# sarphiv/nerf-experiments

Hardware: AMD Instinct MI355X
Metric: ray-samples/sec (coarse+fine), training step (higher is better)
Workload: dtype fp32

## Files before the change

include/nerf_amd.h:

```cpp
#ifndef NERF_AMD_H
#define NERF_AMD_H

#include <stdint.h>
#include <stddef.h>

#ifdef __cplusplus
extern "C" {
#endif

#define NERF_OK 0
#define NERF_ERR_INVALID_ARG (-1)
#define NERF_ERR_UNSUPPORTED (-2)
#define NERF_ERR_LAUNCH (-3)
#define NERF_ERR_WORKSPACE (-4)

int nerf_abi_version(void);
const char* nerf_status_string(int status);
int64_t nerf_struct_size(int32_t which);
#define NERF_BUILD_DIAG_FUSED 1
#define NERF_BUILD_DIAG_WGRAD 2
int32_t nerf_build_flags(void);

int nerf_composite_fwd(const float* density, int64_t density_stride,
                       const float* color, int64_t color_stride,
// ... 145 lines not shown
    float* out2;
    int64_t ldo2;
    int32_t n1;
    int32_t hbm_off;
    int32_t seg_gen[2];
} nerf_fused_layer;

struct nerf_hashgrid_params;
typedef struct nerf_fused_encoding {
    nerf_pe_params params;
    const float* ray_o;
    const float* ray_d;
    const float* t_start;
    const float* t_end;
    const float* pixel_width;
    float* out;
    int64_t ld;
    int64_t n_rays;
    int32_t samples_per_ray;
    int32_t per_ray;
    int32_t out_dim;
    int32_t reserved;
    const struct nerf_hashgrid_params* hash;
    const float* hash_table;
} nerf_fused_encoding;

int nerf_mlp_fused_fwd(const nerf_fused_layer* layers, int32_t n_layers, const void* image, int64_t M,
                       const nerf_fused_encoding* encodings, void* stream);

typedef struct nerf_fused_composite {
    const float* dist;
    float* rgb;
    float* weights;
    float* coef;
    const float* grad_rgb;
    float* grad_head;
    int64_t ld_head;
    float* grad_sigma;
    int64_t ld_sigma;
    int32_t samples_per_ray;
    int32_t head_layer;
    int32_t sigma_layer;
    float scale_a, scale_b;
    float density_shift;
    int32_t reserved;
} nerf_fused_composite;

int nerf_mlp_fused_render(const nerf_fused_layer* layers, int32_t n_layers, const void* image, int64_t M,
                          const nerf_fused_encoding* encodings, const nerf_fused_composite* composite,
                          void* stream);

#define NERF_FUSED_BF16 1
#define NERF_FUSED_SPLIT_OUT(l) (1 << (8 + (l)))
int nerf_mlp_fused_run(const nerf_fused_layer* layers, int32_t n_layers, const void* image, int64_t M,
                       const nerf_fused_encoding* encodings, const nerf_fused_composite* composite, int32_t flags,
                       void* stream);

#define NERF_FUSED_MAX_SRCS 64
int nerf_fused_pack(const float* const* srcs, int32_t n_srcs, const int32_t* map_src, const int32_t* map_dst,
                    int64_t n, void* image, void* stream);

size_t nerf_gauss_act_workspace(int64_t M, int32_t N);

#define NERF_GAUSS_FWD 0
#define NERF_GAUSS_BWD 1
size_t nerf_linear_gauss_workspace(int64_t M, int32_t N);
int nerf_linear_gauss_x3(const nerf_seg* segs, int32_t n_segs, int64_t M, const void* W_x, int32_t ldw,
                         int32_t N, const float* bias, float* out, int64_t ldo, int32_t mode,
                         const float* inv_std, float* y, int64_t ld_y, const float* z, int64_t ld_z,
                         float* grad_inv_std, int32_t accumulate, void* workspace, size_t workspace_bytes,
                         void* stream);
int nerf_gauss_act_fwd(const float* z, int64_t ld_z, const float* inv_std, int64_t M, int32_t N,
                       float* y, int64_t ld_y, void* stream);
int nerf_gauss_act_bwd(const float* grad_y, int64_t ld_g, const float* z, int64_t ld_z,
                       const float* inv_std, int64_t M, int32_t N, float* grad_z, int64_t ld_dz,
                       float* grad_inv_std, int32_t accumulate, void* workspace, size_t workspace_bytes,
                       void* stream);

#define NERF_ACT_GABOR 1
#define NERF_ACT_SARF 2
size_t nerf_param_act_workspace(int32_t kind, int64_t M, int32_t N);
int nerf_param_act_fwd(int32_t kind, const float* z, int64_t ld_z, const float* p0, const float* p1, int64_t M,
                       int32_t N, float* y, int64_t ld_y, void* stream);
int nerf_param_act_bwd(int32_t kind, const float* grad_y, int64_t ld_g, const float* z, int64_t ld_z,
                       const float* p0, const float* p1, int64_t M, int32_t N, float* grad_z, int64_t ld_dz,
                       float* grad_p0, float* grad_p1, int32_t accumulate, void* workspace,
                       size_t workspace_bytes, void* stream);

size_t nerf_linear_act_workspace(int32_t kind, int64_t M, int32_t N);
int nerf_linear_act_x3(int32_t kind, const nerf_seg* segs, int32_t n_segs, int64_t M, const void* W_x, int32_t ldw,
                       int32_t N, const float* bias, float* out, int64_t ldo, int32_t mode, const float* p0,
                       const float* p1, float* y, int64_t ld_y, const float* z, int64_t ld_z, float* grad_p0,
                       float* grad_p1, int32_t accumulate, void* workspace, size_t workspace_bytes, void* stream);

#define NERF_ADAM_MAX_TENSORS 48
typedef struct nerf_adam_batch {
    int32_t n_tensors;
    float beta1, beta2, eps;
    float one_minus_beta1, one_minus_beta2;
    float* param[NERF_ADAM_MAX_TENSORS];
    const float* grad[NERF_ADAM_MAX_TENSORS];
    float* exp_avg[NERF_ADAM_MAX_TENSORS];
    float* exp_avg_sq[NERF_ADAM_MAX_TENSORS];
    int64_t numel[NERF_ADAM_MAX_TENSORS];
    float step_size[NERF_ADAM_MAX_TENSORS];
    float bc2_sqrt[NERF_ADAM_MAX_TENSORS];
// ... 76 lines not shown
```

nerf-experiments_amd/csrc/mlp_fused.hip:

```cpp
#include <stddef.h>
#include <stdlib.h>
#include <string.h>

#include <type_traits>

#include "common.h"
#include "encode_common.h"
#include "composite_common.h"
#include "hashgrid_common.h"

using namespace nerf;

typedef float f4 __attribute__((ext_vector_type(4)));
typedef float f8 __attribute__((ext_vector_type(8)));
typedef __bf16 bf16x8 __attribute__((ext_vector_type(8)));
typedef __bf16 bf16x4 __attribute__((ext_vector_type(4)));

namespace {

typedef __attribute__((address_space(3))) void lds_void_t;
typedef __attribute__((address_space(1))) void glb_void_t;

constexpr int SLOT_BYTES = 16 * 1024;
constexpr int NSLOT = 2;
constexpr int SB = 1;
constexpr int XIMG_BYTES = SB * 16 * 1024;
constexpr int WG = 512 / SB;
constexpr int NWAVE = WG / 64;
constexpr int SPW = 16 * SB;
constexpr int TILE = NWAVE * SPW;
constexpr int KBMAX = 8;
constexpr unsigned OOB = 0x80000000u;
constexpr int RSRC_W3 = 0x00020000;
constexpr int ST_AUX = 2;
constexpr bool is_fwd(int mode) { return (mode & 1) == 0; }
constexpr bool is_x1(int mode) { return (mode & 2) != 0; }
constexpr bool is_qs(int mode) { return (mode & 4) != 0; }
template <int MODE>
constexpr int after_dma_vm() { return is_fwd(MODE) ? 1 + 2 * SB : 2 * SB; }

struct FusedArgs {
    nerf_fused_layer L[NERF_FUSED_MAX_LAYERS];
    nerf_fused_encoding enc[2];
    const char* img;
    int img_bytes;
    int gen_mask;
    int gen_lds;
    int gen_reg;
    int n_layers;
    int M;
    int ntiles;
    int span;
    int comp_on;
    int split_mask;
    nerf_fused_composite comp;
    nerf_hashgrid_params hg;
    const float* hg_table;
    int hg_off[16];
};
static_assert(sizeof(FusedArgs) <= 4096, "kernel arguments");

typedef __attribute__((address_space(4))) const char kchar_t;
typedef float* fptr_t;
typedef const float* cfptr_t;
typedef uint8_t* u8ptr_t;
typedef const uint8_t* cu8ptr_t;
#define LF(T, f, l)                                                                                          \
    (*(const __attribute__((address_space(4))) T*)(c.kargs + offsetof(FusedArgs, L) +                        \
                                                   (size_t)(l) * sizeof(nerf_fused_layer) +                  \
                                                   offsetof(nerf_fused_layer, f)))
#define LFI(T, f, i, l)                                                                                      \
    (*(const __attribute__((address_space(4))) T*)(c.kargs + offsetof(FusedArgs, L) +                        \
                                                   (size_t)(l) * sizeof(nerf_fused_layer) +                  \
                                                   offsetof(nerf_fused_layer, f) + (size_t)(i) * sizeof(T)))

#define EF(T, f, e)                                                                                          \
    (*(const __attribute__((address_space(4))) T*)(c.kargs + offsetof(FusedArgs, enc) +                      \
                                                   (size_t)(e) * sizeof(nerf_fused_encoding) +               \
                                                   offsetof(nerf_fused_encoding, f)))

#define HG(T, f) (*(const __attribute__((address_space(4))) T*)(c.kargs + offsetof(FusedArgs, hg) +               \
                                                               offsetof(nerf_hashgrid_params, f)))

#define CF(T, f)                                                                                             \
    (*(const __attribute__((address_space(4))) T*)(c.kargs + offsetof(FusedArgs, comp) +                    \
                                                   offsetof(nerf_fused_composite, f)))

__device__ __forceinline__ f4 mfma16(bf16x8 a, bf16x8 b, f4 c) {
    return __builtin_amdgcn_mfma_f32_16x16x32_bf16(a, b, c, 0, 0, 0);
}
__device__ __forceinline__ void split8(f8 v, bf16x8& hi, bf16x8& lo) {
    hi = __builtin_convertvector(v, bf16x8);
    lo = __builtin_convertvector(v - __builtin_convertvector(hi, f8), bf16x8);
}

__device__ __forceinline__ void barrier() {
    asm volatile("s_waitcnt lgkmcnt(0)" ::: "memory");
    __builtin_amdgcn_s_barrier();
    __builtin_amdgcn_sched_barrier(0);
}

__device__ __forceinline__ int n16_of(int N) { return (N + 15) >> 4; }

__device__ __forceinline__ unsigned lds_addr(const void* p) {
    return (unsigned)(uintptr_t)(const __attribute__((address_space(3))) char*)p;
}
template <int OFF>
// ... 472 lines not shown
                f4 va, vb;
                unsigned oa, ob;
                pair_stores(c, st, sb, ch, st.colok, st.pa[sb], st.pb[sb], v, va, vb, oa, ob);
                __builtin_amdgcn_raw_buffer_store_b128(va, st.ro, oa, 0, ST_AUX);
                __builtin_amdgcn_raw_buffer_store_b128(vb, st.ro, ob, 0, ST_AUX);
            } else {
                f4 va, vb;
                unsigned oa, ob;
                pair_stores(c, st, sb, ch - st.n1, st.colok2, st.pa2[sb], st.pb2[sb], v, va, vb, oa, ob);
                __builtin_amdgcn_raw_buffer_store_b128(va, st.ro2, oa, 0, ST_AUX);
                __builtin_amdgcn_raw_buffer_store_b128(vb, st.ro2, ob, 0, ST_AUX);
            }
        }
    } else if (p == 2) {
        if constexpr (is_fwd(MODE)) {
            if (ch >= 0 && ch < 2 * KBMAX) {
#pragma unroll
                for (int sb = 0; sb < SB; ++sb) {
                    unsigned t = st.mw[sb][1];
#pragma unroll
                    for (int r = 3; r >= 0; --r) t = shift_in_dead(t, a[sb][r]);
                    st.mw[sb][1] = t;
                }
                if (ch == 7) {
#pragma unroll
                    for (int sb = 0; sb < SB; ++sb) {
                        st.mw[sb][0] = st.mw[sb][1];
                        st.mw[sb][1] = 0;
                    }
                }
            }
        }
    } else {
        if (ch >= 0 && ch < 2 * KBMAX && ch < st.n1 && !(is_qs(MODE) && st.qsplit)) {
#pragma unroll
            for (int sb = 0; sb < SB; ++sb) {
                typedef unsigned u2 __attribute__((ext_vector_type(2)));
                char* d = c.ximg + ((q * SB + sb) * 2) * 1024 + c.lane * 16 + 8 * bb;
                if constexpr (is_x1(MODE)) {
                    *reinterpret_cast<u2*>(d) = u2{hi2(a[sb][0], a[sb][1]), hi2(a[sb][2], a[sb][3])};
                } else {
                    unsigned h0, l0, h1, l1;
                    split2(a[sb][0], a[sb][1], h0, l0);
                    split2(a[sb][2], a[sb][3], h1, l1);
                    const u2 h = {h0, h1}, lo = {l0, l1};
                    *reinterpret_cast<u2*>(d) = h;
                    *reinterpret_cast<u2*>(d + 1024) = lo;
                }
            }
        }
    }
}

constexpr int EPI_NP = 3;
__host__ __device__ constexpr int epi_part_of(int i) {
    return i == 0 ? 0 : i + 1;
}
template <int KBR, int EPI0>
__host__ __device__ constexpr int epi_placed() {
    return KBR - EPI0 < EPI_NP ? (KBR - EPI0 > 0 ? KBR - EPI0 : 0) : EPI_NP;
}

template <int MODE>
constexpr int epi0_of() { return is_fwd(MODE) ? 3 : 4; }

constexpr int FA = 2;

template <int MODE, int KBR, int I>
__device__ __forceinline__ void first_reads(bf16x8 (&fr)[FA][2], unsigned sa) {
    if constexpr (I < FA && I < KBR) {
        lds_frag<I * 2048>(fr[I][0], sa);
        if constexpr (!is_x1(MODE)) lds_frag<I * 2048 + 1024>(fr[I][1], sa);
        first_reads<MODE, KBR, I + 1>(fr, sa);
    }
}

template <int MODE, int KBR, int KBH, int KB_I, int EPAR = -1>
__device__ __forceinline__ void reg_steps(Ctx& c, LayerState& st, unsigned sa, bf16x8 (&fr)[FA][2], f4 (&a)[SB],
                                          f4 (&pv)[SB], f4& pb, int ch) {
    constexpr int EPI0 = KBR >= 8 ? epi0_of<MODE>() : (KBR >= 4 ? 1 : 0);
    if constexpr (KB_I < KBR) {
        bf16x8(&f)[2] = fr[KB_I % FA];
        constexpr int later = (KB_I + FA - 1 < KBR - 1 ? KB_I + FA - 1 : KBR - 1) - KB_I;
        if constexpr (is_x1(MODE)) {
            lds_wait1<later>(f[0]);
#pragma unroll
            for (int sb = 0; sb < SB; ++sb) a[sb] = mfma16(f[0], c.xh[KB_I][sb], a[sb]);
        } else {
            lds_wait<2 * later>(f[0], f[1]);
#pragma unroll
            for (int sb = 0; sb < SB; ++sb) a[sb] = mfma16(f[1], c.xh[KB_I][sb], a[sb]);
#pragma unroll
            for (int sb = 0; sb < SB; ++sb) a[sb] = mfma16(f[0], c.xl[KB_I][sb], a[sb]);
#pragma unroll
            for (int sb = 0; sb < SB; ++sb) a[sb] = mfma16(f[0], c.xh[KB_I][sb], a[sb]);
        }
        if constexpr (KB_I + FA < KBR) {
            lds_frag<(KB_I + FA) * 2048>(f[0], sa);
            if constexpr (!is_x1(MODE)) lds_frag<(KB_I + FA) * 2048 + 1024>(f[1], sa);
        }
        if constexpr (KB_I == EPI0 && is_fwd(MODE))
            bias_wait<(KBR > 0 ? DMA_PER_WAVE : 0) + (is_x1(MODE) ? 1 : 2) * KBH>(pb);
        if constexpr (KB_I >= EPI0 && KB_I < EPI0 + epi_placed<KBR, EPI0>())
            epi_part<MODE, EPAR>(c, st, epi_part_of(KB_I - EPI0), ch - 1, pv, pb);
        __builtin_amdgcn_sched_barrier(0);
        reg_steps<MODE, KBR, KBH, KB_I + 1, EPAR>(c, st, sa, fr, a, pv, pb, ch);
    }
}

template <int MODE, int KBR, int KBH>
__device__ __forceinline__ void fused_layer(Ctx& c, int l, int base) {
    constexpr int EPI0 = KBR >= 8 ? epi0_of<MODE>() : (KBR >= 4 ? 1 : 0);
    const int g = c.lane >> 4;
    const int N = LF(int, N, l);
    const int NC = n16_of(N);
    LayerState st;
    const int ldo = (int)LF(int64_t, ldo, l);
    st.floor_i = LF(int, relu, l) != 0 ? 0 : (int)0x80000000;
    st.qsplit = is_qs(MODE) &&
                ((*(const __attribute__((address_space(4))) int*)(c.kargs + offsetof(FusedArgs, split_mask)) >> l) & 1) != 0;
    st.colok = ldo - 4 * g;
    st.last_even = (NC & 1) ? NC - 1 : -1;
    int sample[SB];
    bool row_ok[SB];
#pragma unroll
    for (int sb = 0; sb < SB; ++sb) {
        sample[sb] = base + 16 * sb + (c.lane & 15);
        row_ok[sb] = sample[sb] < c.M;
        st.row_off[sb] = row_ok[sb] ? (unsigned)sample[sb] * (unsigned)ldo * 4u + 16u * g : OOB;
        st.sample_off[sb] = row_ok[sb] && g == 0 ? (unsigned)sample[sb] * 4u : OOB;
        st.mrow_off[sb] = row_ok[sb] ? (unsigned)sample[sb] * 32u + 8u * g : OOB;
        {
            const int sa = (c.lane & 8) == 0 ? sample[sb] : sample[sb] - 8;
            const int sbb = sa + 8;
            st.pa[sb] = sa < c.M ? (unsigned)sa * (unsigned)ldo * 4u + 16u * g : OOB;
            st.pb[sb] = sbb < c.M ? (unsigned)sbb * (unsigned)ldo * 4u + 16u * g : OOB;
        }
        st.mw[sb][0] = st.mw[sb][1] = 0;
    }
    st.ro = __builtin_amdgcn_make_buffer_rsrc(LF(fptr_t, out, l), 0, c.M * ldo * 4, RSRC_W3);
    st.bias_off = (unsigned)LF(int64_t, bias_off, l) + 16u * g;
    if constexpr (is_fwd(MODE)) {
        uint8_t* mptr = LF(u8ptr_t, mask, l);
        st.rm = __builtin_amdgcn_make_buffer_rsrc(mptr, 0, mptr != nullptr ? c.M * 32 : 0, RSRC_W3);
        float* cptr = LF(fptr_t, col_out, l);
        st.col_chunk = cptr != nullptr ? LF(int, col_idx, l) / 16 : -1;
        st.rc = __builtin_amdgcn_make_buffer_rsrc(cptr, 0, cptr ? c.M * 4 : 0, RSRC_W3);
        st.n1 = NC;
    } else {
        float* o2 = LF(fptr_t, out2, l);
        st.n1 = o2 != nullptr ? 2 * LF(int, n1, l) : NC;
        const int ldo2 = o2 != nullptr ? (int)LF(int64_t, ldo2, l) : 0;
        st.colok2 = ldo2 - 4 * g;
        st.ro2 = __builtin_amdgcn_make_buffer_rsrc(o2, 0, o2 ? c.M * ldo2 * 4 : 0, RSRC_W3);
#pragma unroll
        for (int sb = 0; sb < SB; ++sb)
            st.row_off2[sb] = row_ok[sb] ? (unsigned)sample[sb] * (unsigned)ldo2 * 4u + 16u * g : OOB;
#pragma unroll
        for (int sb = 0; sb < SB; ++sb) {
            const int sa = (c.lane & 8) == 0 ? sample[sb] : sample[sb] - 8;
            const int sbb = sa + 8;
            st.pa2[sb] = sa < c.M ? (unsigned)sa * (unsigned)ldo2 * 4u + 16u * g : OOB;
            st.pb2[sb] = sbb < c.M ? (unsigned)sbb * (unsigned)ldo2 * 4u + 16u * g : OOB;
        }
        const uint8_t* mi = LF(cu8ptr_t, mask_in, l);
        const __amdgpu_buffer_rsrc_t rmi =
            __builtin_amdgcn_make_buffer_rsrc(const_cast<uint8_t*>(mi), 0, mi != nullptr ? c.M * 32 : 0, RSRC_W3);
#pragma unroll
        for (int sb = 0; sb < SB; ++sb) {
            const unsigned off = st.mrow_off[sb];
            typedef unsigned u2 __attribute__((ext_vector_type(2)));
            const u2 w = __builtin_bit_cast(u2, __builtin_amdgcn_raw_buffer_load_b64(rmi, off, 0, 0));
            st.mi[sb][0] = w.x;
            st.mi[sb][1] = w.y;
            st.mcur[sb] = w.x;
        }
    }

    bf16x8 hh[KBH > 0 ? KBH : 1][SB], hl[KBH > 0 ? KBH : 1][SB];
    if constexpr (KBH > 0) {
        const int kb0 = LFI(int, seg_kb, 0, l);
#pragma unroll
        for (int kh = 0; kh < KBH; ++kh) {
            const int sg = kh < kb0 ? 0 : 1;
            const int khl = sg ? kh - kb0 : kh;
            const int gen = sg ? LFI(int, seg_gen, 1, l) : LFI(int, seg_gen, 0, l);
            if (!is_fwd(MODE) && gen >= 3) {
                comp_grad_block(c, gen, sg ? LFI(cfptr_t, seg_ptr, 1, l) : LFI(cfptr_t, seg_ptr, 0, l), sample,
                                row_ok, hh[kh], hl[kh]);
                continue;
            }
            if (is_fwd(MODE) && gen != 0) {
                if constexpr (KBR == 0) {
#pragma unroll
                    for (int sb = 0; sb < SB; ++sb)
                        gen_block(c, 16 * sb + (c.lane & 15), 32 * khl + 8 * g, hh[kh][sb], hl[kh][sb]);
                } else {
#pragma unroll
                    for (int sb = 0; sb < SB; ++sb) {
                        hh[kh][sb] = c.gh[sb];
                        hl[kh][sb] = c.gl[sb];
                    }
                }
                continue;
            }
            const float* p = sg ? LFI(cfptr_t, seg_ptr, 1, l) : LFI(cfptr_t, seg_ptr, 0, l);
            const int64_t ld = sg ? LFI(int64_t, seg_ld, 1, l) : LFI(int64_t, seg_ld, 0, l);
            const int k = sg ? LFI(int, seg_k, 1, l) : LFI(int, seg_k, 0, l);
            const int rd = sg ? LFI(int, seg_rd, 1, l) : LFI(int, seg_rd, 0, l);
            const int rows = sg ? LFI(int, seg_rows, 1, l) : LFI(int, seg_rows, 0, l);
            const __amdgpu_buffer_rsrc_t rs =
                __builtin_amdgcn_make_buffer_rsrc(const_cast<float*>(p), 0, (int)((int64_t)rows * ld * 4), RSRC_W3);
            const int col = 32 * khl + 8 * g;
#pragma unroll
            for (int sb = 0; sb < SB; ++sb) {
                const unsigned m = (unsigned)(row_ok[sb] ? sample[sb] : 0);
                const unsigned row = rd == 1 ? m : m / (unsigned)rd;
                const unsigned rbase = (unsigned)(((int64_t)row * ld + col) * 4);
                const f4 x0 = __builtin_amdgcn_raw_buffer_load_b128(rs, col < k ? rbase : OOB, 0, 0);
                const f4 x1 = __builtin_amdgcn_raw_buffer_load_b128(rs, col + 4 < k ? rbase + 16 : OOB, 0, 0);
                split8(__builtin_shufflevector(x0, x1, 0, 1, 2, 3, 4, 5, 6, 7), hh[kh][sb], hl[kh][sb]);
            }
        }
    }
    if constexpr (KBH > 0) {
#pragma unroll
        for (int kh = 0; kh < KBH; ++kh)
#pragma unroll
            for (int sb = 0; sb < SB; ++sb) {
                if constexpr (is_x1(MODE))
                    asm volatile("" : "+v"(hh[kh][sb]));
                else
                    asm volatile("" : "+v"(hh[kh][sb]), "+v"(hl[kh][sb]));
            }
    }
    const unsigned hbm_frag = (unsigned)LF(int, hbm_off, l) + (unsigned)c.lane * 16u;

    f4 pv[SB] = {};
    if constexpr (KBR == 0) {
        typedef bf16x8 fragk_t[KBH > 0 ? KBH : 1][2];
        auto frag_load = [&](fragk_t& f, int ch) __attribute__((always_inline)) {
#pragma unroll
            for (int kh = 0; kh < KBH; ++kh)
#pragma unroll
                for (int hl_ = 0; hl_ < (is_x1(MODE) ? 1 : 2); ++hl_)
                    f[kh][hl_] = __builtin_bit_cast(
                        bf16x8, __builtin_amdgcn_raw_buffer_load_b128(
                                    c.rimg, hbm_frag + (unsigned)(((ch * KBH + kh) * 2 + hl_) * 1024), 0, 0));
        };
        auto bias_load = [&](int ch) __attribute__((always_inline)) {
            return __builtin_bit_cast(f4, __builtin_amdgcn_raw_buffer_load_b128(
                                              c.rimg, st.bias_off + (is_fwd(MODE) ? 64u * (unsigned)ch : 0u), 0, 0));
        };
        fragk_t hA, hB;
        f4 bA, bB = f4{0.f, 0.f, 0.f, 0.f};
        frag_load(hA, 0);
        auto step = [&](int ch, fragk_t& cur, fragk_t& nxt, f4& bthis, const f4& bprev) __attribute__((always_inline)) {
            frag_load(nxt, ch + 1 < NC ? ch + 1 : ch);
            bthis = bias_load(ch);
            f4 a[SB];
#pragma unroll
            for (int sb = 0; sb < SB; ++sb) a[sb] = f4{0.f, 0.f, 0.f, 0.f};
#pragma unroll
            for (int kh = 0; kh < KBH; ++kh) {
                if constexpr (!is_x1(MODE)) {
#pragma unroll
                    for (int sb = 0; sb < SB; ++sb) a[sb] = mfma16(cur[kh][1], hh[kh][sb], a[sb]);
#pragma unroll
                    for (int sb = 0; sb < SB; ++sb) a[sb] = mfma16(cur[kh][0], hl[kh][sb], a[sb]);
                }
#pragma unroll
                for (int sb = 0; sb < SB; ++sb) a[sb] = mfma16(cur[kh][0], hh[kh][sb], a[sb]);
            }
#pragma unroll
            for (int i = 0; i < EPI_NP; ++i) epi_part<MODE>(c, st, epi_part_of(i), ch - 1, pv, bprev);
#pragma unroll
            for (int sb = 0; sb < SB; ++sb) pv[sb] = a[sb];
        };
        for (int ch = 0; ch < NC; ch += 2) {
            step(ch, hA, hB, bA, bB);
            if (ch + 1 < NC) step(ch + 1, hB, hA, bB, bA);
        }
    } else
    {
    auto chunk = [&](int ch, auto ep_tag) __attribute__((always_inline)) {
        constexpr int EP = decltype(ep_tag)::value;
        f4 pb = {0.f, 0.f, 0.f, 0.f};
        if constexpr (is_fwd(MODE))
            buf_load16(pb, st.bias_off + 64u * (unsigned)(ch > 0 ? ch - 1 : 0), c.rimg);
        const unsigned sa = lds_addr(c.smem + c.cur * SLOT_BYTES + c.lane * 16);
        bf16x8 fr[FA][2];
        if constexpr (KBR > 0) {
            asm volatile("s_waitcnt vmcnt(%0)" ::"n"(after_dma_vm<MODE>()) : "memory");
#ifndef NERF_FUSED_DIAG_NOBARRIER
            barrier();
#endif
#ifdef NERF_FUSED_DIAG_BAR2
            barrier();
#endif
            first_reads<MODE, KBR, 0>(fr, sa);
            issue_dma(c, c.cur ^ 1);
            __builtin_amdgcn_sched_barrier(0);
        }
        bf16x8 hf[KBH > 0 ? KBH : 1][2];
#pragma unroll
        for (int kh = 0; kh < KBH; ++kh)
#pragma unroll
            for (int hl_ = 0; hl_ < (is_x1(MODE) ? 1 : 2); ++hl_)
                buf_load16(hf[kh][hl_], hbm_frag + (unsigned)(((ch * KBH + kh) * 2 + hl_) * 1024), c.rimg);
        f4 a[SB];
#pragma unroll
        for (int sb = 0; sb < SB; ++sb) a[sb] = f4{0.f, 0.f, 0.f, 0.f};
        reg_steps<MODE, KBR, KBH, 0, EP>(c, st, sa, fr, a, pv, pb, ch);
#pragma unroll
        for (int kh = 0; kh < KBH; ++kh) {
            if constexpr (is_x1(MODE))
                frag_vwait1<(KBR > 0 ? 2 * SB : 0)>(hf[kh][0]);
            else
                frag_vwait<(KBR > 0 ? 2 * SB : 0)>(hf[kh][0], hf[kh][1]);
        }
#pragma unroll
        for (int kh = 0; kh < KBH; ++kh) {
            if constexpr (!is_x1(MODE)) {
#pragma unroll
                for (int sb = 0; sb < SB; ++sb) a[sb] = mfma16(hf[kh][1], hh[kh][sb], a[sb]);
#pragma unroll
                for (int sb = 0; sb < SB; ++sb) a[sb] = mfma16(hf[kh][0], hl[kh][sb], a[sb]);
            }
#pragma unroll
            for (int sb = 0; sb < SB; ++sb) a[sb] = mfma16(hf[kh][0], hh[kh][sb], a[sb]);
            __builtin_amdgcn_sched_barrier(0);
        }
        if constexpr (KBR == 0) bias_wait<0>(pb);
#pragma unroll
        for (int i = epi_placed<KBR, EPI0>(); i < EPI_NP; ++i) epi_part<MODE, EP>(c, st, epi_part_of(i), ch - 1, pv, pb);
        if constexpr (KBR > 0) c.cur ^= 1;
#pragma unroll
        for (int sb = 0; sb < SB; ++sb) pv[sb] = a[sb];
    };
    for (int ch = 0; ch < NC; ch += 2) {
        chunk(ch, std::integral_constant<int, 1>{});
        if (ch + 1 < NC) chunk(ch + 1, std::integral_constant<int, 0>{});
    }
    }
    {
        f4 lb = {0.f, 0.f, 0.f, 0.f};
        if constexpr (is_fwd(MODE)) {
            buf_load16(lb, st.bias_off + 64u * (unsigned)(NC - 1), c.rimg);
            bias_wait<0>(lb);
        }
#pragma unroll
        for (int p = 0; p < 4; ++p) epi_part<MODE>(c, st, p, NC - 1, pv, lb);
    }
    if constexpr (is_fwd(MODE)) {
        const int nb = NC < 2 * KBMAX ? NC : 2 * KBMAX;
        if (nb < 8) {
#pragma unroll
            for (int sb = 0; sb < SB; ++sb) {
                st.mw[sb][0] = st.mw[sb][1] << (4 * (8 - nb));
                st.mw[sb][1] = 0;
            }
        } else if (nb > 8) {
#pragma unroll
            for (int sb = 0; sb < SB; ++sb) st.mw[sb][1] <<= 4 * (16 - nb);
        }
        typedef unsigned u2 __attribute__((ext_vector_type(2)));
#pragma unroll
        for (int sb = 0; sb < SB; ++sb)
            __builtin_amdgcn_raw_buffer_store_b64(u2{st.mw[sb][0], st.mw[sb][1]}, st.rm, st.mrow_off[sb], 0, 0);
    }
    if constexpr (is_fwd(MODE)) {
#pragma unroll
        for (int sb = 0; sb < SB; ++sb) c.head[sb] = pv[sb];
    }
    if (l + 1 == c.n_layers) return;
#pragma unroll
    for (int kb = 0; kb < KBMAX; ++kb)
#pragma unroll
        for (int sb = 0; sb < SB; ++sb) {
            c.xh[kb][sb] = *reinterpret_cast<const bf16x8*>(c.ximg + ((kb * SB + sb) * 2) * 1024 + c.lane * 16);
            c.xl[kb][sb] = *reinterpret_cast<const bf16x8*>(c.ximg + ((kb * SB + sb) * 2 + 1) * 1024 + c.lane * 16);
        }
}

constexpr int COMP_OFF = 8192;
constexpr int COMP_SMAX = 2 * TILE;
constexpr int COMP_DEL = COMP_SMAX * 16;
static_assert(COMP_OFF >= SB * 2048 && COMP_OFF + COMP_SMAX * 20 <= XIMG_BYTES, "composite scratch");

template <int R, class CT>
__device__ __forceinline__ void composite_wave(CT& c, int64_t ray, int S, int roff = 0) {
    const char* reg = c.ximg + COMP_OFF + roff;
    float rd[R], del[R], rc[R][3];
#pragma unroll
    for (int r = 0; r < R; ++r) {
        const int s = r * 64 + c.lane;
        rd[r] = 0.f; del[r] = 0.f;
        rc[r][0] = rc[r][1] = rc[r][2] = 0.f;
        if (s < S) {
            const f4 h = *reinterpret_cast<const f4*>(reg + s * 16);
            rc[r][0] = h[0]; rc[r][1] = h[1]; rc[r][2] = h[2]; rd[r] = h[3];
            del[r] = *reinterpret_cast<const float*>(reg + COMP_DEL + s * 4);
        }
    }
    float w[R], rgb[3], cc[R][3], cs[R][3];
// ... 249 lines not shown
            n = 256;
    }
    return n;
}

}

namespace {
int enc_out_dim(const nerf_pe_params& p) { return (2 * p.levels + (p.include_identity ? 1 : 0)) * 3; }

bool hash_ok(const nerf_fused_encoding& e) {
    const nerf_hashgrid_params* h = e.hash;
    if (h == nullptr || e.hash_table == nullptr || !aligned16(e.hash_table)) return false;
    if (h->levels < 1 || h->levels > 16 || !(h->features == 1 || h->features == 2 || h->features == 4)) return false;
    if (h->table_size < 1 || (int64_t)h->levels * h->table_size * h->features >= ((int64_t)1 << 31)) return false;
    if (!(h->normalize == 0 || h->normalize == 1) || !(h->query == 0 || h->query == 1)) return false;
    if (e.params.query != h->query || e.per_ray || e.out_dim != h->levels * h->features) return false;
    for (int l = 0; l < h->levels; ++l)
        if (h->res[l] < 1 || h->res[l] > (1 << 20)) return false;
    return true;
}

bool encoding_ok(const nerf_fused_encoding& e, int64_t M) {
    const nerf_pe_params& p = e.params;
    if (p.kind == 2) {
        if (!hash_ok(e)) return false;
    } else if (!(p.levels >= 0 && p.levels <= 16 && (p.kind == 0 || p.kind == 1))) {
        return false;
    }
    if ((p.kind != 2 && e.out_dim != enc_out_dim(p)) || e.out_dim <= 0 || e.samples_per_ray < 1 || e.n_rays < 1)
        return false;
    if (e.n_rays * e.samples_per_ray < M || M >= ((int64_t)1 << 31)) return false;
    if (e.ray_d == nullptr) return false;
    if (e.per_ray) {
        if (p.kind != 0) return false;
    } else {
        if (e.ray_o == nullptr || e.t_start == nullptr || (p.query != 0 && e.t_end == nullptr)) return false;
        if (p.kind == 1 && (e.t_end == nullptr || e.pixel_width == nullptr || p.pw_mode < 0 || p.pw_mode > 2))
            return false;
    }
    if (e.out != nullptr) {
        const int64_t rows = e.per_ray ? e.n_rays : M;
        if (!aligned16(e.out) || e.ld % 4 != 0 || e.ld < e.out_dim || rows * e.ld * 4 >= ((int64_t)1 << 31))
            return false;
    }
    return true;
}
}

namespace {
int fused_launch(const nerf_fused_layer* layers, int32_t n_layers, const void* image, int64_t M,
                 const nerf_fused_encoding* encodings, const nerf_fused_composite* comp, int32_t flags, void* stream) {
    const int split_mask = (int)(((uint32_t)flags >> 8) & 0xffffu);
    NERF_REQUIRE((flags & ~(NERF_FUSED_BF16 | (0xffff << 8))) == 0);
    const bool single_pass = (flags & NERF_FUSED_BF16) != 0;
    NERF_REQUIRE(layers != nullptr && image != nullptr);
    NERF_REQUIRE(n_layers >= 1 && n_layers <= NERF_FUSED_MAX_LAYERS);
    NERF_REQUIRE(M >= 1 && M <= (int64_t)1 << 30);
    FusedArgs a;
    int64_t img_end = 0;
    int gen_lds = -1, gen_reg = -1;
    bool dgrad = false;
    for (int l = 0; l < n_layers; ++l) dgrad = dgrad || layers[l].mask_in != nullptr || layers[l].out2 != nullptr;
    for (int l = 0; l < n_layers; ++l) {
        if (dgrad)
            NERF_REQUIRE(layers[l].relu == 0 && layers[l].mask == nullptr && layers[l].col_out == nullptr);
    }
    NERF_REQUIRE((split_mask >> n_layers) == 0 && (split_mask == 0 || (!dgrad && !single_pass)));
    for (int l = 0; l < n_layers; ++l)
        if ((split_mask >> l) & 1)
            NERF_REQUIRE(l < n_layers - 1 && layers[l].N <= 256 && layers[l].col_out == nullptr &&
                         layers[l].out != nullptr);
    for (int l = 0; l < n_layers; ++l) {
        const nerf_fused_layer& L = layers[l];
        const int kbr = (L.type / 3) * 4, kbh = L.type % 3;
        NERF_REQUIRE(L.type == 1 || L.type == 2 || L.type == 3 || L.type == 6 || L.type == 7 || L.type == 8);
        NERF_REQUIRE((l == 0) == (kbr == 0));
        NERF_REQUIRE(L.N >= 1 && L.nb == (L.N + 31) / 32 && L.nb <= 16);
        const int n16 = (L.N + 15) / 16;
        NERF_REQUIRE(L.chunk_units == 2 * kbr);
        NERF_REQUIRE(L.img_off >= 0 && L.img_off % 1024 == 0);
        NERF_REQUIRE(L.hbm_off >= 0 && L.hbm_off % 1024 == 0);
        NERF_REQUIRE(L.bias_off >= 0 && L.bias_off % 16 == 0);
        img_end = img_end > L.img_off + (int64_t)n16 * 2048 * kbr ? img_end : L.img_off + (int64_t)n16 * 2048 * kbr;
        img_end = img_end > (int64_t)L.hbm_off + (int64_t)n16 * 2048 * kbh ? img_end
                                                                          : (int64_t)L.hbm_off + (int64_t)n16 * 2048 * kbh;
        img_end = img_end > L.bias_off + 64 * n16 ? img_end : L.bias_off + 64 * n16;
        NERF_REQUIRE((L.out == nullptr && L.ldo == 0) ||
                     (L.out != nullptr && aligned16(L.out) && L.ldo % 4 == 0 &&
                      L.ldo >= (L.out2 != nullptr ? (32 * L.n1 < L.N ? 32 * L.n1 : L.N) : L.N)));
        NERF_REQUIRE(M * L.ldo * 4 < ((int64_t)1 << 31));
        NERF_REQUIRE(L.mask == nullptr || (L.N <= 256 && M * 32 < ((int64_t)1 << 31)));
        NERF_REQUIRE(L.mask_in == nullptr || M * 32 < ((int64_t)1 << 31));
        NERF_REQUIRE(L.col_out == nullptr || (L.col_idx >= 0 && L.col_idx % 32 == 0 && L.col_idx < L.N));
        NERF_REQUIRE(L.out2 == nullptr || (aligned16(L.out2) && L.ldo2 % 4 == 0 && L.ldo2 > 0 && L.n1 >= 0 &&
                                           L.n1 <= L.nb && M * L.ldo2 * 4 < ((int64_t)1 << 31)));
        NERF_REQUIRE(L.nseg >= 0 && L.nseg <= 2);
        int kbs = 0;
        for (int s = 0; s < 2; ++s) {
            const int gen = s < L.nseg ? L.seg_gen[s] : 0;
            NERF_REQUIRE(s < L.nseg || L.seg_gen[s] == 0);
            if (gen == 0) continue;
            if (gen >= 3) {
                NERF_REQUIRE(dgrad && gen <= 4 && comp != nullptr && comp->grad_rgb != nullptr && L.nseg == 1);
                NERF_REQUIRE(L.seg_kb[0] == 1 && L.seg_k[0] == 8 && L.seg_ld[0] == 8 && L.seg_rd[0] == 1);
                NERF_REQUIRE(L.seg_ptr[0] != nullptr && aligned16(L.seg_ptr[0]) && L.seg_rows[0] >= M);
                NERF_REQUIRE((int64_t)L.seg_rows[0] * 32 < ((int64_t)1 << 31));
// ... 39 lines not shown
    NERF_REQUIRE(img_end < ((int64_t)1 << 31));
    int gen_mask = 0;
    memset(&a.hg, 0, sizeof(a.hg));
    a.hg_table = nullptr;
    memset(a.hg_off, 0, sizeof(a.hg_off));
    for (int e = 0; e < 2; ++e) {
        if (encodings != nullptr && encodings[e].out_dim > 0) {
            NERF_REQUIRE(!dgrad && encoding_ok(encodings[e], M) && encodings[e].out != nullptr && encodings[e].ld <= 64);
            a.enc[e] = encodings[e];
            gen_mask |= 1 << e;
            if (encodings[e].params.kind == 2) {
                NERF_REQUIRE(a.hg_table == nullptr);
                a.hg = *encodings[e].hash;
                a.hg_table = encodings[e].hash_table;
                int64_t off = 0;
                for (int l = 0; l < a.hg.levels; ++l) {
                    a.hg_off[l] = (int)off;
                    off += level_rows(a.hg.res[l], a.hg.table_size);
                }
            }
        } else {
            memset(&a.enc[e], 0, sizeof(a.enc[e]));
        }
    }
    NERF_REQUIRE(gen_lds < 0 || ((gen_mask >> gen_lds) & 1));
    NERF_REQUIRE(gen_reg < 0 || ((gen_mask >> gen_reg) & 1));
    for (int l = 0; l < n_layers && gen_mask != 0; ++l) {
        const nerf_fused_layer& L = layers[l];
        for (int s = 0; s < L.nseg; ++s) {
            if (L.seg_gen[s] != 0) continue;
            const char* p = static_cast<const char*>(static_cast<const void*>(L.seg_ptr[s]));
            const char* pe = p + (int64_t)L.seg_rows[s] * L.seg_ld[s] * 4;
            for (int e = 0; e < 2; ++e) {
                if (!((gen_mask >> e) & 1)) continue;
                const nerf_fused_encoding& E = encodings[e];
                const char* q = static_cast<const char*>(static_cast<const void*>(E.out));
                const char* qe = q + (E.per_ray ? E.n_rays : M) * E.ld * 4;
                if (p < qe && q < pe)
                    NERF_REQUIRE((!E.per_ray || E.samples_per_ray == 1) && L.seg_rd[s] == 1 && p == q && L.seg_ld[s] == E.ld);
            }
        }
    }
    a.gen_mask = gen_mask;
    a.gen_lds = gen_lds;
    a.gen_reg = gen_reg;
    a.img = static_cast<const char*>(image);
    a.img_bytes = (int)img_end;
    a.n_layers = n_layers;
    a.M = (int)M;
    a.ntiles = (int)((M + TILE - 1) / TILE);
    a.span = 1;
    a.comp_on = 0;
    a.split_mask = split_mask;
    memset(&a.comp, 0, sizeof(a.comp));
    if (comp != nullptr) {
        a.comp = *comp;
        const int S = comp->samples_per_ray;
        if (!dgrad) {
            NERF_REQUIRE(((S >= 16 && S <= TILE && TILE % S == 0 && TILE / S <= NWAVE) || S == 2 * TILE) &&
                         M % S == 0);
            if (S == 2 * TILE) a.span = 2;
            NERF_REQUIRE(comp->dist != nullptr && comp->rgb != nullptr);
            NERF_REQUIRE(comp->coef == nullptr || (aligned16(comp->coef) && M * 32 < ((int64_t)1 << 31)));
            const nerf_fused_layer& H = layers[n_layers - 1];
            NERF_REQUIRE(comp->head_layer == n_layers - 1 && H.type >= 3 && H.N <= 16);
            NERF_REQUIRE(H.N >= (comp->sigma_layer < 0 ? 4 : 3));
            NERF_REQUIRE(comp->sigma_layer < n_layers - 1);
            if (comp->sigma_layer >= 0) NERF_REQUIRE(layers[comp->sigma_layer].col_out != nullptr);
            a.comp_on = 1;
        }
    }
    const int ngroups = a.ntiles / a.span;
    const int grid = ngroups < num_cus() ? ngroups : num_cus();
    if (single_pass) {
        if (dgrad)
            hipLaunchKernelGGL(mlp_fused_kernel<MODE_DGRAD | MODE_X1>, dim3(grid), dim3(WG), 0, as_stream(stream), a);
        else
            hipLaunchKernelGGL(mlp_fused_kernel<MODE_FWD | MODE_X1>, dim3(grid), dim3(WG), 0, as_stream(stream), a);
    } else if (dgrad) {
        hipLaunchKernelGGL(mlp_fused_kernel<MODE_DGRAD>, dim3(grid), dim3(WG), 0, as_stream(stream), a);
    } else if (split_mask != 0) {
        hipLaunchKernelGGL(mlp_fused_kernel<MODE_FWD | MODE_QS>, dim3(grid), dim3(WG), 0, as_stream(stream), a);
    } else {
        hipLaunchKernelGGL(mlp_fused_kernel<MODE_FWD>, dim3(grid), dim3(WG), 0, as_stream(stream), a);
    }
    NERF_CHECK_LAUNCH();
    return NERF_OK;
}
}

extern "C" int nerf_mlp_fused_fwd(const nerf_fused_layer* layers, int32_t n_layers, const void* image, int64_t M,
                                  const nerf_fused_encoding* encodings, void* stream) {
    return fused_launch(layers, n_layers, image, M, encodings, nullptr, 0, stream);
}

extern "C" int nerf_mlp_fused_render(const nerf_fused_layer* layers, int32_t n_layers, const void* image, int64_t M,
                                     const nerf_fused_encoding* encodings, const nerf_fused_composite* composite,
                                     void* stream) {
    return fused_launch(layers, n_layers, image, M, encodings, composite, 0, stream);
}

extern "C" int nerf_mlp_fused_run(const nerf_fused_layer* layers, int32_t n_layers, const void* image, int64_t M,
                                  const nerf_fused_encoding* encodings, const nerf_fused_composite* composite,
                                  int32_t flags, void* stream) {
    return fused_launch(layers, n_layers, image, M, encodings, composite, flags, stream);
}
// ... 19 lines not shown
```

nerf-experiments_amd/nerf_amd/_lib.py:

```python
from __future__ import annotations

import ctypes
import os

import torch

_HERE = os.path.dirname(os.path.abspath(__file__))
LIB_PATH = os.environ.get("NERF_AMD_LIB", os.path.join(_HERE, "libnerf_amd.so"))

c_f = ctypes.c_float
c_i32 = ctypes.c_int32
c_i64 = ctypes.c_int64
c_u32 = ctypes.c_uint32
c_u64 = ctypes.c_uint64
c_vp = ctypes.c_void_p
c_sz = ctypes.c_size_t

NERF_EPI_BIAS = 1
NERF_EPI_RELU = 2
NERF_EPI_MASK = 4
NERF_EPI_ACCUM = 8
NERF_EPI_MASKBITS = 16
NERF_EPI_MASKOUT = 32
NERF_EPI_NO_PERSIST = 256
NERF_EPI_NARROW_TILE = 512
NERF_EPI_TANH = 4096
NERF_EPI_TANH_BWD = 8192
NERF_ERR_UNSUPPORTED = -2
NERF_FUSED_BF16 = 1


def NERF_FUSED_SPLIT_OUT(layer: int) -> int:
    return 1 << (8 + layer)

NERF_KABSCH_MAX_POINTS = 4096
NERF_PROP_MAX_EDGES = 512
NERF_GAUSS_FWD = 0
NERF_GAUSS_BWD = 1
NERF_ACT_GABOR = 1
NERF_ACT_SARF = 2


class NerfSeg(ctypes.Structure):
    _fields_ = [("ptr", c_vp), ("ld", c_i64), ("k", c_i32), ("row_div", c_i32)]


class NerfPEParams(ctypes.Structure):
    _fields_ = [
        ("kind", c_i32),
        ("levels", c_i32),
        ("include_identity", c_i32),
        ("query", c_i32),
        ("scale", c_f),
        ("pixel_width_sigma", c_f),
        ("distribute_variance", c_i32),
        ("pw_mode", c_i32),
        ("use_mask", c_i32),
        ("mask", c_f * 16),
    ]


NERF_ADAM_MAX_TENSORS = 48


class NerfAdamBatch(ctypes.Structure):
    _fields_ = [
        ("n_tensors", c_i32),
        ("beta1", c_f),
        ("beta2", c_f),
        ("eps", c_f),
        ("one_minus_beta1", c_f),
        ("one_minus_beta2", c_f),
        ("param", c_vp * NERF_ADAM_MAX_TENSORS),
        ("grad", c_vp * NERF_ADAM_MAX_TENSORS),
        ("exp_avg", c_vp * NERF_ADAM_MAX_TENSORS),
        ("exp_avg_sq", c_vp * NERF_ADAM_MAX_TENSORS),
        ("numel", c_i64 * NERF_ADAM_MAX_TENSORS),
        ("step_size", c_f * NERF_ADAM_MAX_TENSORS),
        ("bc2_sqrt", c_f * NERF_ADAM_MAX_TENSORS),
        ("weight_decay", c_f * NERF_ADAM_MAX_TENSORS),
    ]

# ... 224 lines not shown
```

nerf-experiments_amd/nerf_amd/mlp_fused.py:

```python
from __future__ import annotations

import ctypes
import os

import numpy as np
import torch

from . import _lib
from . import kernels as K

def _pack_image(f) -> None:
    ps = []
    for lp in f.plan.layers:
        ps += [lp.module.weight, lp.module.bias]
    arr = (ctypes.c_void_p * len(ps))(*[p.detach().contiguous().data_ptr() for p in ps])
    st = _lib.load().nerf_fused_pack(arr, len(ps), f.map_src.data_ptr(), f.map_dst.data_ptr(), f.map_src.numel(),
                                     f.image.data_ptr(), K._stream(f.device))
    _lib.check(st, "nerf_fused_pack")


def _flags(passes: int) -> int:
    if passes not in (1, 3):
        raise ValueError(f"fused MLP: passes must be 1 or 3 (got {passes})")
    return _lib.NERF_FUSED_BF16 if passes == 1 else 0


FUSED_TYPES = {(0, 1): 1, (0, 2): 2, (4, 0): 3, (8, 0): 6, (8, 1): 7, (8, 2): 8}
ENABLED = os.environ.get("NERF_FUSED", "1") != "0"
CAPTURE_PER_RAY = os.environ.get("NERF_FUSED_CAPTURE", "1") != "0"


def _layer_shape(plan, idx):
    lp = plan.layers[idx]
    if lp.pact or lp.tanh or lp.residual >= 0:
        return None
    acts = [s for s in lp.sources if s.kind == "act"]
    hbm = [s for s in lp.sources if s.kind != "act"]
    if idx == 0:
        if acts:
            return None
        kbr = 0
    else:
        if len(acts) != 1 or lp.sources[0] is not acts[0] or acts[0].layer != idx - 1:
            return None
        if acts[0].k_valid not in (128, 256):
            return None
        kbr = acts[0].k_valid // 32
    if len(hbm) > 2 or any(s.kind not in ("pos", "dir") for s in hbm):
        return None
    kbh = sum(s.k_pad // 32 for s in hbm)
    if (kbr, kbh) not in FUSED_TYPES:
        return None
    return kbr, hbm


def eligible(plan, M: int) -> bool:
    if not ENABLED or len(plan.layers) > _lib.NERF_FUSED_MAX_LAYERS or M >= (1 << 30):
        return False
    if len(plan.layers) * 2 > _lib.NERF_FUSED_MAX_SRCS:
        return False
    cols = {}
    for li, c in plan.column_outputs:
        if c % 32 or li in cols:
            return False
        cols[li] = c
    for idx, lp in enumerate(plan.layers):
        if _layer_shape(plan, idx) is None:
            return False
        N = lp.module.out_features
        if (N + 31) // 32 > 9 or M * lp.out_ld * 4 >= (1 << 31):
            return False
        if idx + 1 < len(plan.layers) and plan.layers[idx + 1].sources[0].kind == "act" and N > 288:
            return False
    return True


def _fragment_maps(n16, kbr, kbh, row_of, red_reg, red_hbm, elem, img_off, hbm_off, bias_off, bias_code):
    lane = np.arange(64)
    srow = lane & 15
# ... 387 lines not shown
```

Baseline: 70.47 million.

## Add specialized plain-layer epilogue path for register-fed hidden layers in fused MLP

Adds a streamlined epilogue (epi_plain) and chunk schedule for hidden layers that take register-fed inputs only, have a contiguous output and no extra outputs. These layers skip the generic epilogue branches, use a tighter vmcnt wait and a reworked bias-load and epilogue placement across chunk pairs. A GENERIC flag lets callers fall back to the old path. This adds code size and register pressure and carries correctness risk in the hand-scheduled waitcnts.

```diff
diff --git a/include/nerf_amd.h b/include/nerf_amd.h
--- a/include/nerf_amd.h
+++ b/include/nerf_amd.h
@@ -221,6 +221,7 @@
 
 #define NERF_FUSED_BF16 1
 #define NERF_FUSED_SPLIT_OUT(l) (1 << (8 + (l)))
+#define NERF_FUSED_GENERIC 2
 int nerf_mlp_fused_run(const nerf_fused_layer* layers, int32_t n_layers, const void* image, int64_t M,
                        const nerf_fused_encoding* encodings, const nerf_fused_composite* composite, int32_t flags,
                        void* stream);
diff --git a/nerf-experiments_amd/csrc/mlp_fused.hip b/nerf-experiments_amd/csrc/mlp_fused.hip
--- a/nerf-experiments_amd/csrc/mlp_fused.hip
+++ b/nerf-experiments_amd/csrc/mlp_fused.hip
@@ -53,6 +53,7 @@
     int span;
     int comp_on;
     int split_mask;
+    int no_plain;
     nerf_fused_composite comp;
     nerf_hashgrid_params hg;
     const float* hg_table;
@@ -631,6 +632,110 @@
     }
 }
 
+template <int MODE, int EPAR>
+__device__ __forceinline__ void epi_plain(Ctx& c, LayerState& st, int p, int ch, f4 (&a)[SB], f4 b) {
+    static_assert(EPAR == 0 || EPAR == 1, "compile-time parity");
+    const int q = ch >> 1;
+    constexpr int bb = EPAR;
+    if (p < 2) {
+        if (p >= SB) return;
+        const int sb = p;
+        f4& v = a[sb];
+        if constexpr (is_fwd(MODE)) {
+#pragma unroll
+            for (int r = 0; r < 4; ++r)
+                v[r] = __builtin_bit_cast(float, max(__builtin_bit_cast(int, v[r] + b[r]), st.floor_i));
+            f4 sv = v;
+            if constexpr (is_qs(MODE)) {
+                if (st.qsplit) {
+                    typedef unsigned u2 __attribute__((ext_vector_type(2)));
+                    typedef unsigned u4 __attribute__((ext_vector_type(4)));
+                    unsigned h0, l0, h1, l1;
+                    split2(v[0], v[1], h0, l0);
+                    split2(v[2], v[3], h1, l1);
+                    char* d = c.ximg + ((q * SB + sb) * 2) * 1024 + c.lane * 16 + 8 * bb;
+                    *reinterpret_cast<u2*>(d) = u2{h0, h1};
+                    *reinterpret_cast<u2*>(d + 1024) = u2{l0, l1};
+                    sv = __builtin_bit_cast(f4, u4{h0, h1, l0, l1});
+                }
+            }
+            if constexpr (EPAR == 0) {
+                st.stash[sb] = sv;
+            } else {
+                const int so = 64 * (ch - 1);
+                __builtin_amdgcn_raw_buffer_store_b128(st.stash[sb], st.ro, st.row_off[sb], so, ST_AUX);
+                __builtin_amdgcn_raw_buffer_store_b128(sv, st.ro, st.row_off[sb] + 64u, so, ST_AUX);
+            }
+        } else {
+            const int sh = 4 * (7 - (ch & 7));
+            if constexpr (EPAR == 0) {
+                if (ch == 8) st.mcur[sb] = st.mi[sb][1];
+            }
+#pragma unroll
+            for (int r = 0; r < 4; ++r) {
+                const int dead = __builtin_amdgcn_sbfe((int)st.mcur[sb], (unsigned)(sh + r), 1u);
+                const float x = v[r];
+                v[r] = __builtin_bit_cast(float, __builtin_bit_cast(int, x) & ~dead);
+            }
+            if constexpr (EPAR == 0) {
+                st.stash[sb] = v;
+            } else {
+                const f4 x = st.stash[sb];
+                const bool lo8 = (c.lane & 8) == 0;
+                f4 rx, ry;
+#pragma unroll
+                for (int r = 0; r < 4; ++r) {
+                    const float xr = x[r], yr = v[r];
+                    rx[r] = ror8(xr);
+                    ry[r] = ror8(yr);
+                }
+                const f4 va = lo8 ? x : ry;
+                const f4 vb = lo8 ? rx : v;
+                const int so = 64 * (ch - 1);
+                __builtin_amdgcn_raw_buffer_store_b128(va, st.ro, st.pa[sb], so, ST_AUX);
+                __builtin_amdgcn_raw_buffer_store_b128(vb, st.ro, st.pb[sb], so, ST_AUX);
+            }
+        }
+    } else if (p == 2) {
+        if constexpr (is_fwd(MODE)) {
+#pragma unroll
+            for (int sb = 0; sb < SB; ++sb) {
+                unsigned t = st.mw[sb][1];
+#pragma unroll
+                for (int r = 3; r >= 0; --r) t = shift_in_dead(t, a[sb][r]);
+                st.mw[sb][1] = t;
+            }
+            if constexpr (EPAR == 1) {
+                if (ch == 7) {
+#pragma unroll
+                    for (int sb = 0; sb < SB; ++sb) {
+                        st.mw[sb][0] = st.mw[sb][1];
+                        st.mw[sb][1] = 0;
+                    }
+                }
+            }
+        }
+    } else {
+        if (!(is_qs(MODE) && st.qsplit)) {
+#pragma unroll
+            for (int sb = 0; sb < SB; ++sb) {
+                typedef unsigned u2 __attribute__((ext_vector_type(2)));
+                char* d = c.ximg + ((q * SB + sb) * 2) * 1024 + c.lane * 16 + 8 * bb;
+                if constexpr (is_x1(MODE)) {
+                    *reinterpret_cast<u2*>(d) = u2{hi2(a[sb][0], a[sb][1]), hi2(a[sb][2], a[sb][3])};
+                } else {
+                    unsigned h0, l0, h1, l1;
+                    split2(a[sb][0], a[sb][1], h0, l0);
+                    split2(a[sb][2], a[sb][3], h1, l1);
+                    const u2 h = {h0, h1}, lo = {l0, l1};
+                    *reinterpret_cast<u2*>(d) = h;
+                    *reinterpret_cast<u2*>(d + 1024) = lo;
+                }
+            }
+        }
+    }
+}
+
 constexpr int EPI_NP = 3;
 __host__ __device__ constexpr int epi_part_of(int i) {
     return i == 0 ? 0 : i + 1;
@@ -654,7 +759,7 @@
     }
 }
 
-template <int MODE, int KBR, int KBH, int KB_I, int EPAR = -1>
+template <int MODE, int KBR, int KBH, int KB_I, int EPAR = -1, bool PL = false>
 __device__ __forceinline__ void reg_steps(Ctx& c, LayerState& st, unsigned sa, bf16x8 (&fr)[FA][2], f4 (&a)[SB],
                                           f4 (&pv)[SB], f4& pb, int ch) {
     constexpr int EPI0 = KBR >= 8 ? epi0_of<MODE>() : (KBR >= 4 ? 1 : 0);
@@ -678,12 +783,16 @@
             lds_frag<(KB_I + FA) * 2048>(f[0], sa);
             if constexpr (!is_x1(MODE)) lds_frag<(KB_I + FA) * 2048 + 1024>(f[1], sa);
         }
-        if constexpr (KB_I == EPI0 && is_fwd(MODE))
+        if constexpr (KB_I == EPI0 && is_fwd(MODE) && !(PL && EPAR == 2))
             bias_wait<(KBR > 0 ? DMA_PER_WAVE : 0) + (is_x1(MODE) ? 1 : 2) * KBH>(pb);
-        if constexpr (KB_I >= EPI0 && KB_I < EPI0 + epi_placed<KBR, EPI0>())
-            epi_part<MODE, EPAR>(c, st, epi_part_of(KB_I - EPI0), ch - 1, pv, pb);
+        if constexpr (KB_I >= EPI0 && KB_I < EPI0 + epi_placed<KBR, EPI0>()) {
+            if constexpr (!PL)
+                epi_part<MODE, EPAR>(c, st, epi_part_of(KB_I - EPI0), ch - 1, pv, pb);
+            else if constexpr (EPAR != 2)
+                epi_plain<MODE, EPAR>(c, st, epi_part_of(KB_I - EPI0), ch - 1, pv, pb);
+        }
         __builtin_amdgcn_sched_barrier(0);
-        reg_steps<MODE, KBR, KBH, KB_I + 1, EPAR>(c, st, sa, fr, a, pv, pb, ch);
+        reg_steps<MODE, KBR, KBH, KB_I + 1, EPAR, PL>(c, st, sa, fr, a, pv, pb, ch);
     }
 }
 
@@ -756,6 +865,25 @@
         }
     }
 
+    bool plain = false;
+    if constexpr (KBR == 8 && KBH == 0) {
+        plain = NERF_TU_BUILD_FLAGS == 0 &&
+                *(const __attribute__((address_space(4))) int*)(c.kargs + offsetof(FusedArgs, no_plain)) == 0 &&
+                (N & 31) == 0 && N <= 32 * KBMAX && ldo == N &&
+                LF(fptr_t, out, l) != nullptr &&
+                (is_fwd(MODE) ? LF(fptr_t, col_out, l) == nullptr : LF(fptr_t, out2, l) == nullptr);
+        if constexpr (!is_fwd(MODE)) {
+            if (plain) {
+#pragma unroll
+                for (int sb = 0; sb < SB; ++sb) {
+                    const unsigned hi8 = (c.lane & 8) != 0 ? 64u : 0u;
+                    st.pa[sb] += hi8;
+                    st.pb[sb] += hi8;
+                }
+            }
+        }
+    }
+
     bf16x8 hh[KBH > 0 ? KBH : 1][SB], hl[KBH > 0 ? KBH : 1][SB];
     if constexpr (KBH > 0) {
         const int kb0 = LFI(int, seg_kb, 0, l);
@@ -816,6 +944,20 @@
     const unsigned hbm_frag = (unsigned)LF(int, hbm_off, l) + (unsigned)c.lane * 16u;
 
     f4 pv[SB] = {};
+    auto last_epilogue = [&](auto pl_tag) __attribute__((always_inline)) {
+        f4 lb = {0.f, 0.f, 0.f, 0.f};
+        if constexpr (is_fwd(MODE)) {
+            buf_load16(lb, st.bias_off + 64u * (unsigned)(NC - 1), c.rimg);
+            bias_wait<0>(lb);
+        }
+#pragma unroll
+        for (int p = 0; p < 4; ++p) {
+            if constexpr (decltype(pl_tag)::value)
+                epi_plain<MODE, 1>(c, st, p, NC - 1, pv, lb);
+            else
+                epi_part<MODE>(c, st, p, NC - 1, pv, lb);
+        }
+    };
     if constexpr (KBR == 0) {
         typedef bf16x8 fragk_t[KBH > 0 ? KBH : 1][2];
         auto frag_load = [&](fragk_t& f, int ch) __attribute__((always_inline)) {
@@ -860,17 +1002,21 @@
             step(ch, hA, hB, bA, bB);
             if (ch + 1 < NC) step(ch + 1, hB, hA, bB, bA);
         }
+        last_epilogue(std::false_type{});
     } else
     {
-    auto chunk = [&](int ch, auto ep_tag) __attribute__((always_inline)) {
+    auto chunk = [&](int ch, auto ep_tag, auto vm_tag) __attribute__((always_inline)) {
         constexpr int EP = decltype(ep_tag)::value;
+        constexpr int VM = decltype(vm_tag)::value;
+        constexpr bool PL = VM >= 0;
+        static_assert(!PL || (KBR == 8 && KBH == 0), "plain layers: register-fed only");
         f4 pb = {0.f, 0.f, 0.f, 0.f};
-        if constexpr (is_fwd(MODE))
-            buf_load16(pb, st.bias_off + 64u * (unsigned)(ch > 0 ? ch - 1 : 0), c.rimg);
+        if constexpr (is_fwd(MODE) && !(PL && EP == 2))
+            buf_load16(pb, st.bias_off + 64u * (unsigned)(PL || ch > 0 ? ch - 1 : 0), c.rimg);
         const unsigned sa = lds_addr(c.smem + c.cur * SLOT_BYTES + c.lane * 16);
         bf16x8 fr[FA][2];
         if constexpr (KBR > 0) {
-            asm volatile("s_waitcnt vmcnt(%0)" ::"n"(after_dma_vm<MODE>()) : "memory");
+            asm volatile("s_waitcnt vmcnt(%0)" ::"n"(PL ? VM : after_dma_vm<MODE>()) : "memory");
 #ifndef NERF_FUSED_DIAG_NOBARRIER
             barrier();
 #endif
@@ -890,7 +1036,7 @@
         f4 a[SB];
 #pragma unroll
         for (int sb = 0; sb < SB; ++sb) a[sb] = f4{0.f, 0.f, 0.f, 0.f};
-        reg_steps<MODE, KBR, KBH, 0, EP>(c, st, sa, fr, a, pv, pb, ch);
+        reg_steps<MODE, KBR, KBH, 0, EP, PL>(c, st, sa, fr, a, pv, pb, ch);
 #pragma unroll
         for (int kh = 0; kh < KBH; ++kh) {
             if constexpr (is_x1(MODE))
@@ -912,24 +1058,36 @@
         }
         if constexpr (KBR == 0) bias_wait<0>(pb);
 #pragma unroll
-        for (int i = epi_placed<KBR, EPI0>(); i < EPI_NP; ++i) epi_part<MODE, EP>(c, st, epi_part_of(i), ch - 1, pv, pb);
+        for (int i = epi_placed<KBR, EPI0>(); i < EPI_NP; ++i) {
+            if constexpr (!PL) epi_part<MODE, EP>(c, st, epi_part_of(i), ch - 1, pv, pb);
+        }
         if constexpr (KBR > 0) c.cur ^= 1;
 #pragma unroll
         for (int sb = 0; sb < SB; ++sb) pv[sb] = a[sb];
     };
-    for (int ch = 0; ch < NC; ch += 2) {
-        chunk(ch, std::integral_constant<int, 1>{});
-        if (ch + 1 < NC) chunk(ch + 1, std::integral_constant<int, 0>{});
-    }
-    }
-    {
-        f4 lb = {0.f, 0.f, 0.f, 0.f};
-        if constexpr (is_fwd(MODE)) {
-            buf_load16(lb, st.bias_off + 64u * (unsigned)(NC - 1), c.rimg);
-            bias_wait<0>(lb);
-        }
-#pragma unroll
-        for (int p = 0; p < 4; ++p) epi_part<MODE>(c, st, p, NC - 1, pv, lb);
+    auto generic_loop = [&]() __attribute__((always_inline)) {
+        for (int ch = 0; ch < NC; ch += 2) {
+            chunk(ch, std::integral_constant<int, 1>{}, std::integral_constant<int, -1>{});
+            if (ch + 1 < NC) chunk(ch + 1, std::integral_constant<int, 0>{}, std::integral_constant<int, -1>{});
+        }
+        last_epilogue(std::false_type{});
+    };
+    if constexpr (KBR == 8 && KBH == 0) {
+        if (plain) {
+            constexpr int V_LO = is_fwd(MODE) ? 1 : 0, V_HI = is_fwd(MODE) ? 3 : 2;
+            chunk(0, std::integral_constant<int, 2>{}, std::integral_constant<int, V_HI>{});
+            chunk(1, std::integral_constant<int, 0>{}, std::integral_constant<int, V_LO>{});
+            for (int ch = 2; ch < NC; ch += 2) {
+                chunk(ch, std::integral_constant<int, 1>{}, std::integral_constant<int, V_LO>{});
+                chunk(ch + 1, std::integral_constant<int, 0>{}, std::integral_constant<int, V_HI>{});
+            }
+            last_epilogue(std::true_type{});
+        } else {
+            generic_loop();
+        }
+    } else {
+        generic_loop();
+    }
     }
     if constexpr (is_fwd(MODE)) {
         const int nb = NC < 2 * KBMAX ? NC : 2 * KBMAX;
@@ -1285,7 +1443,7 @@
 int fused_launch(const nerf_fused_layer* layers, int32_t n_layers, const void* image, int64_t M,
                  const nerf_fused_encoding* encodings, const nerf_fused_composite* comp, int32_t flags, void* stream) {
     const int split_mask = (int)(((uint32_t)flags >> 8) & 0xffffu);
-    NERF_REQUIRE((flags & ~(NERF_FUSED_BF16 | (0xffff << 8))) == 0);
+    NERF_REQUIRE((flags & ~(NERF_FUSED_BF16 | NERF_FUSED_GENERIC | (0xffff << 8))) == 0);
     const bool single_pass = (flags & NERF_FUSED_BF16) != 0;
     NERF_REQUIRE(layers != nullptr && image != nullptr);
     NERF_REQUIRE(n_layers >= 1 && n_layers <= NERF_FUSED_MAX_LAYERS);
@@ -1431,6 +1589,7 @@
     a.span = 1;
     a.comp_on = 0;
     a.split_mask = split_mask;
+    a.no_plain = (flags & NERF_FUSED_GENERIC) != 0;
     memset(&a.comp, 0, sizeof(a.comp));
     if (comp != nullptr) {
         a.comp = *comp;
diff --git a/nerf-experiments_amd/nerf_amd/_lib.py b/nerf-experiments_amd/nerf_amd/_lib.py
--- a/nerf-experiments_amd/nerf_amd/_lib.py
+++ b/nerf-experiments_amd/nerf_amd/_lib.py
@@ -28,6 +28,7 @@
 NERF_EPI_TANH_BWD = 8192
 NERF_ERR_UNSUPPORTED = -2
 NERF_FUSED_BF16 = 1
+NERF_FUSED_GENERIC = 2
 
 
 def NERF_FUSED_SPLIT_OUT(layer: int) -> int:
diff --git a/nerf-experiments_amd/nerf_amd/mlp_fused.py b/nerf-experiments_amd/nerf_amd/mlp_fused.py
--- a/nerf-experiments_amd/nerf_amd/mlp_fused.py
+++ b/nerf-experiments_amd/nerf_amd/mlp_fused.py
@@ -22,9 +22,10 @@
 def _flags(passes: int) -> int:
     if passes not in (1, 3):
         raise ValueError(f"fused MLP: passes must be 1 or 3 (got {passes})")
-    return _lib.NERF_FUSED_BF16 if passes == 1 else 0
-
-
+    return (_lib.NERF_FUSED_BF16 if passes == 1 else 0) | (_lib.NERF_FUSED_GENERIC if FORCE_GENERIC else 0)
+
+
+FORCE_GENERIC = False
 FUSED_TYPES = {(0, 1): 1, (0, 2): 2, (4, 0): 3, (8, 0): 6, (8, 1): 7, (8, 2): 8}
 ENABLED = os.environ.get("NERF_FUSED", "1") != "0"
 CAPTURE_PER_RAY = os.environ.get("NERF_FUSED_CAPTURE", "1") != "0"
```

Result: faster. 72.12 million (median of 6 runs) (+2.3%).
